# srtee/lammps-USER-CONP2

Measured on AMD Instinct MI355X. Metric: charge-solve updates/sec + ns/day, 4096-atom electrode / 32k electrolyte, higher is better.
Workload: dtype f64; 1 GPU; synthetic graphene/IL 4096 electrode + 32768 electrolyte, ffield; Ne=4096, Nl=32768, K=99773, kflat=645, mode=ffield, solver=inv, kspace=ewald, blist_pairs=302717, structure_factor_form=z-window (32 columns, grid 480)

## Files before the change

### include/conp_hip.h

```cpp
#ifndef CONP_HIP_H
#define CONP_HIP_H

#include <stddef.h>
#include <stdint.h>

#ifdef __cplusplus
extern "C" {
#endif

#define CONP_ABI_VERSION 1

typedef enum {
  CONP_OK = 0,
  CONP_ERR_ARG = -1,
  CONP_ERR_STATE = -2,
  CONP_ERR_NO_DEVICE = -3,
  CONP_ERR_NUMERIC = -4,
  CONP_ERR_IO = -5
} conp_status;

enum { CONP_FF_NORMAL = 0, CONP_FF_FFIELD = 1, CONP_FF_NOSLAB = 2 };
enum { CONP_SOLVER_CG = 0, CONP_SOLVER_INV = 1 };

typedef struct conp_fix conp_fix;
// ... 128 lines not shown
int conp_compute_potential_atom(conp_fix *fix, const conp_atoms *atoms, const conp_neighlist *pairlist, const int *sel,
                                const int *etasel , const conp_potential_args *args, double *potential);

typedef struct {
  int elenum, elenum_all, elytenum, maxtag_all, runstage;
  int kcount, kcount_flat, kcount_expand, kxmax, kymax, kzmax, kmax, kmax3d;
  int kcount_dims[7];
  int cg_iterations;
  int n_zclasses;
  double unitk[3], volume, gsqmx, ug_tot, totsetq, scalar_output, totinve, slabcorr;
  int64_t n_blist_pairs, n_alist_pairs, n_elyte_charged;
  int inverse_path;
  int inverse_retries;
  int pppm_elyte_spreads;
  int zn_cols, zn_grid, zn_rows;
} conp_info;
int conp_fix_info(const conp_fix *fix, conp_info *out);
int conp_fix_get_ktables(const conp_fix *fix, int *kxvecs, int *kyvecs, int *kzvecs, double *ug, int *kxy_list, int *kz_list);
int conp_fix_get_maps(const conp_fix *fix, int *ele2tag, int *ele2eleall, int *eleall2tag, int *eleall2ele,
                      int *elecheck_eleall, int *elebuf2eleall, int *tag2eleall);
int conp_fix_get_matrix(conp_fix *fix, double *aaa_all );
int conp_fix_set_matrix(conp_fix *fix, const double *aaa_all, int runstage);
int conp_fix_get_vectors(conp_fix *fix, double *bbb_all, double *eleallq, double *elesetq);
int conp_fix_get_sfac(conp_fix *fix, double *sfacrl, double *sfacim);
int conp_fix_get_ele_trig(conp_fix *fix, double *csk, double *snk);
int conp_inv_project(conp_fix *fix, int n, double *aaa, int nullneutral, int zneutr, const double *eleallz, double zhalf,
                     double *totinve_out);

int conp_fix_write_matrix_file(conp_fix *fix, const char *path, int which);
int conp_fix_read_matrix_file(conp_fix *fix, const conp_atoms *atoms, const char *path);
// ... 69 lines not shown
void conp_host_free(void *p);

int conp_debug_check_guards(void);

enum {
  CONP_PATH_PARTIAL_TILES = 1 << 0,
  CONP_PATH_A_GENERAL = 1 << 1,
  CONP_PATH_INV_PIVOTED = 1 << 2,
  CONP_PATH_CG_TWO_LAUNCH = 1 << 3,
  CONP_PATH_GEMV_ROWS = 1 << 4,
  CONP_PATH_PHASE_LAUNCH = 1 << 5,
  CONP_PATH_PPPM_SPREAD_LAUNCH = 1 << 6,
  CONP_PATH_ROWS_HOST = 1 << 7,
  CONP_PATH_TIME_SPLIT = 1 << 8,
  CONP_PATH_SK_CLASSIC = 1 << 12,
  CONP_PATH_ZN_WIDE = 1 << 13
};
void conp_debug_set_paths(unsigned mask);
void conp_debug_set_sk_workgroups(int n);
void conp_debug_set_ew_block(int n);


int conp_fix_write_timing(conp_fix *fix);
const char *conp_fix_log_drain(conp_fix *fix);
const char *conp_fix_mesg_drain(conp_fix *fix);

#ifdef __cplusplus
}
#endif
#endif
```

### lammps-user-conp2_amd/conp_amd/capi.py

```python
from __future__ import annotations

import ctypes as C
import os
from typing import Optional, Sequence

import numpy as np

from . import systems as _systems

HERE = os.path.dirname(os.path.abspath(__file__))
_LIB = None


class ConpError(RuntimeError):
    def __init__(self, code, msg):
        super().__init__(f"[conp status {code}] {msg}")
        self.code = code
        self.msg = msg


def library_path():
    return os.environ.get("CONP_LIB") or os.path.join(HERE, "libconp_hip.so")


# ... 49 lines not shown


class conp_pair_build_args(C.Structure):
    _fields_ = [("nlocal", C.c_int), ("nall", C.c_int), ("cutneigh", C.c_double), ("d_tag", C.c_void_p), ("d_nspecial", C.c_void_p),
                ("d_special", C.c_void_p), ("maxspecial", C.c_int), ("prd_half", C.c_double * 3)]


class conp_info(C.Structure):
    _fields_ = [("elenum", C.c_int), ("elenum_all", C.c_int), ("elytenum", C.c_int), ("maxtag_all", C.c_int),
                ("runstage", C.c_int), ("kcount", C.c_int), ("kcount_flat", C.c_int), ("kcount_expand", C.c_int),
                ("kxmax", C.c_int), ("kymax", C.c_int), ("kzmax", C.c_int), ("kmax", C.c_int), ("kmax3d", C.c_int),
                ("kcount_dims", C.c_int * 7), ("cg_iterations", C.c_int), ("n_zclasses", C.c_int), ("unitk", C.c_double * 3),
                ("volume", C.c_double), ("gsqmx", C.c_double), ("ug_tot", C.c_double), ("totsetq", C.c_double),
                ("scalar_output", C.c_double), ("totinve", C.c_double), ("slabcorr", C.c_double),
                ("n_blist_pairs", C.c_int64), ("n_alist_pairs", C.c_int64), ("n_elyte_charged", C.c_int64),
                ("inverse_path", C.c_int), ("inverse_retries", C.c_int), ("pppm_elyte_spreads", C.c_int), ("zn_cols", C.c_int), ("zn_grid", C.c_int), ("zn_rows", C.c_int)]


SYMBOLS = [
    "conp_parse_fix_args", "conp_fix_create", "conp_fix_destroy", "conp_last_error", "conp_abi_version",
    "conp_fix_init_list", "conp_fix_setup_post_neighbor", "conp_fix_setup_pre_force", "conp_fix_post_neighbor",
    "conp_fix_pre_force", "conp_fix_compute_scalar", "conp_fix_post_force", "conp_fix_post_force_step", "conp_fix_modify_param", "conp_fix_linalg_setup", "conp_fix_a_cal", "conp_fix_b_cal",
    "conp_fix_equation_solve", "conp_fix_update_charge", "conp_km_conp_setup", "conp_km_a_cal", "conp_km_b_cal",
    "conp_fix_info", "conp_fix_get_ktables", "conp_fix_get_maps", "conp_fix_get_matrix", "conp_fix_set_matrix",
    "conp_fix_get_vectors", "conp_fix_get_sfac", "conp_fix_get_ele_trig", "conp_inv_project", "conp_invert",
    "conp_host_ktables", "conp_host_index", "conp_host_pair_rows", "conp_fix_write_matrix_file", "conp_fix_read_matrix_file",
    "conp_fix_set_stream",
    "conp_fix_bind_device_buffers", "conp_fix_row_range", "conp_fix_b_cal_device", "conp_fix_solve_device",
    "conp_fix_scatter_device", "conp_fix_pre_force_device", "conp_fix_profile", "conp_fix_profile_read", "conp_debug_check_guards",
    "conp_debug_set_paths", "conp_debug_set_sk_workgroups", "conp_debug_set_ew_block",
    "conp_fix_pin_host_arrays", "conp_fix_unpin_host_arrays", "conp_host_alloc", "conp_host_free",
# ... 4 lines not shown
    "conp_ewald_compute", "conp_ewald_compute_group_potential", "conp_ewald_compute_particle_potential",
    "conp_ewald_compute_forces", "conp_pppm_compute_forces",
    "conp_ewald_compute_forces_device", "conp_pppm_compute_forces_device",
    "conp_ewald_compute_forces_vatom", "conp_pppm_compute_forces_vatom",
    "conp_ewald_compute_forces_vatom_device", "conp_pppm_compute_forces_vatom_device",
    "conp_compute_potential_atom",
    "conp_pair_set_params", "conp_pair_set_list", "conp_pair_compute", "conp_pair_compute_device",
    "conp_pair_build_list_device", "conp_pair_list_moved_device", "conp_pair_get_list",
]


PATH_PARTIAL_TILES, PATH_A_GENERAL, PATH_INV_PIVOTED, PATH_CG_TWO_LAUNCH, PATH_GEMV_ROWS = 1, 2, 4, 8, 16
PATH_PHASE_LAUNCH, PATH_PPPM_SPREAD_LAUNCH, PATH_ROWS_HOST, PATH_TIME_SPLIT = 32, 64, 128, 256
PATH_SK_CLASSIC = 4096
PATH_ZN_WIDE = 8192


class test_paths:

    def __init__(self, mask=0, sk_workgroups=0):
        self.mask, self.nwg = mask, sk_workgroups

    def __enter__(self):
        lib = load_library()
        if not hasattr(lib, "conp_debug_set_paths"):
            raise RuntimeError("this library build has no test hooks (a comparison build of an earlier round?)")
        lib.conp_debug_set_paths(self.mask)
        lib.conp_debug_set_sk_workgroups(self.nwg)
        return self

# ... 690 lines not shown
```

### lammps-user-conp2_amd/csrc/conp_fix.cpp

```cpp
#include <hip/hip_runtime.h>
#include <dlfcn.h>
#include <rccl/rccl.h>

#include <algorithm>
#include <cmath>
#include <cstdarg>
#include <chrono>
#include <cstdio>
#include <cstdlib>
#include <cstring>
#include <map>
#include <memory>
#include <mutex>
#include <stdexcept>
#include <string>
#include <vector>

#include "../../include/conp_hip.h"
#include "conp_host.hpp"
#include "conp_kernels.h"

namespace {

thread_local std::string g_last_error;
// ... 687 lines not shown
  bool zn_listed = false;
  bool zn_off = false;
  bool zn_tables_current = false;
  int zn_n = 0, zn_ncf = 2;
  double zn_gscale = 0.0, zn_beta = 0.0;
  std::vector<ZnItem> zn_items_h;
  DevBuf<ZnItem> d_zn_items;
  DevBuf<int> d_zn_g0c, d_zn_frag_ptr;
  DevBuf<int2> d_zn_frag_ents;
  DevBuf<double> d_zn_P, d_zn_phihat, d_zn_Bt, d_zn_pieces, d_zn_grid, d_zn_Dt;
  DevBuf<int> d_zn_cov_ptr;
  DevBuf<int2> d_zn_cov_ent;
  int zn_nrg = 0;
  DevBuf<double2> d_zn_cs;
  int zn_nfrag = 0;
  std::vector<int> zn_ch_lo, zn_ch_hi;
  int zn_c_start = 0;
  int *zn_flag_host = nullptr, *zn_flag_dev = nullptr;
  bool zn_eligible() const { return !decomposed && !args.pppm && nl >= zn_min_atoms && !path_on(CONP_PATH_SK_CLASSIC); }
  bool zn_use() const { return zn_listed && !zn_off && zn_eligible() && sk_projects() && nzc > 0; }
  bool zn_gen_use() const { return zn_listed && !zn_off && zn_eligible() && !sk_projects() && nzc == 0 && env.nranks <= 1 && zn_nrg > 0; }
  double zn_lz() const { return kt.slabflag ? env.zprd * env.slab_volfactor : env.zprd; }
  void zn_order_list(const conp_atoms *at) {
    zn_listed = false; zn_off = false;
    if (getenv("CONP_TIME_REN")) std::fprintf(stderr, "  z-window: eligible %d (decomposed %d pppm %d nl %d) plan.nz %d\n", (int)zn_eligible(), (int)decomposed, args.pppm, nl, plan.nz);
    if (!zn_eligible() || plan.nz <= 0) return;
    int n = std::max(64, (38 * plan.nz / 10 + 15) / 16 * 16);
    zn_n = n;
    zn_beta = 0.97 * 3.14159265358979323846 * ZN_W * (1.0 - (double)plan.nz / n);
    const double lz = zn_lz();
// ... 85 lines not shown
          if (pos[x] < per_xcd[x].size()) zn_items_h.push_back(by_slot[per_xcd[x][pos[x]++]]);
          else {
            int best = -1; size_t left = 0;
            for (int y = 0; y < 8; ++y) if (per_xcd[y].size() - pos[y] > left) { left = per_xcd[y].size() - pos[y]; best = y; }
            if (best >= 0) zn_items_h.push_back(by_slot[per_xcd[best][pos[best]++]]);
          }
    }
    zn_nfrag = 4 * plan.n_row_tiles;
    std::vector<std::vector<int2>> of_frag(zn_nfrag);
    for (const ZnItem &it : zn_items_h)
      for (int f = 0; f < 4; ++f) of_frag[4 * it.rt + f].push_back(make_int2(it.slot * sk_hc_stride() + 16 * f, 4));
    std::vector<int> fptr(zn_nfrag + 1, 0);
    std::vector<int2> fent;
    for (int g = 0; g < zn_nfrag; ++g) { fent.insert(fent.end(), of_frag[g].begin(), of_frag[g].end()); fptr[g + 1] = (int)fent.size(); }
    if (fent.empty()) fent.push_back(make_int2(0, 4));
    zn_nrg = nrg;
    if (nzc == 0) {
      const int ncol = 16 * zn_ncf;
      std::vector<int> cptr(n + 1, 0);
      std::vector<int2> cent;
      for (int g = 0; g < n; ++g) {
        for (int r = 0; r < nrg; ++r) {
          int col = (g - g0c[ranges[r].first]) % n;
          if (col < 0) col += n;
          if (col < ncol) cent.push_back(make_int2(r, col));
        }
        cptr[g + 1] = (int)cent.size();
      }
      if (cent.empty()) cent.push_back(make_int2(0, 0));
      ren_upload(d_zn_cov_ptr, cptr);
// ... 1014 lines not shown
        prof.begin("elyte_phase", stream);
        ZnWindow zw{};
        const bool zn_now = zn_use() || zn_gen_use();
        if (zn_now) zw = ZnWindow{d_zn_Bt.p, d_zn_g0c.p, zn_flag_dev, 16 * zn_ncf, zn_n, ZN_W, zn_beta, zn_gscale};
        launch_elyte_phase(stream, nl, nl_pad, eidx, ex, eq, kt.unitk[0], kt.unitk[1], kt.unitk[2], plan.kxmax,
                           plan.kymax, plan.nz, plan.kzt, 1 + plan.n_col_tiles * 32, d_Xt.p, d_Yt.p, d_Zt.p, d_qc.p, d_slab_part.p,
                           &n_slab_part, ride && !ride_hc ? &pairs : nullptr, d_breal.p, 16 * table_c0, 16 * table_c1, zn_now ? &zw : nullptr);
        zs_current = !zn_now; last_ex = ex; last_eq = eq; last_eidx = eidx;
        prof.end(stream);
        pairs_keep = pairs;
      }
      fin = make_brow(ne, ne_pad, rr0, rr1, d_b_rowptr.p, d_b_ele.p, d_b_oth.p, dx, dq, d_type.p, real_params(), 1, d_bk.p, slab,
                      d_ele_z.p, d_slab_part.p, n_slab_part, 4.0 * 3.14159265358979323846 / kt.volume, d_b, d_scalars.p + 2);
      fin.breal = d_breal.p;
      use_fin = ride && nzc > 0 && zc_final_fits((int)own_rt_h.size(), nzc);
      const bool proj = sk_projects();
      if (zn_use() && !fuse_phase) {
        zn_ensure_tables();
        prof.begin("zn_gemm", stream);
        launch_zn_gemm(stream, dplan, zn_ncf, d_zn_items.p, (int)zn_items_h.size(), d_Xt.p, d_Yt.p, d_zn_Bt.p, d_zn_P.p, zn_n, nzc,
                       d_zn_pieces.p, sk_hc_stride());
        prof.end(stream);
        g_current = false;
        prof.begin("reduce_project", stream);
        launch_project_zclass_pieces(stream, dplan, ne_pad, (int)own_rt_h.size(), d_own_rt.p, nzc, d_zn_pieces.p, d_hslot_ptr.p, d_hslot_idx.p,
                                     true, d_zn_frag_ptr.p, d_zn_frag_ents.p, zn_nfrag, d_Rp.p, d_Xe.p, d_Ye.p, d_own_pv.p, d_zclass.p, d_Hc.p,
                                     d_bk.p, use_fin ? &fin : nullptr, ride_hc ? &pairs_keep : nullptr, d_breal.p,
                                     zn_nrg > 32 );
        prof.end(stream);
      } else if (zn_gen_use() && !fuse_phase) {
        zn_ensure_tables();
        prof.begin("zn_gemm", stream);
        launch_zn_gemm(stream, dplan, zn_ncf, d_zn_items.p, (int)zn_items_h.size(), d_Xt.p, d_Yt.p, d_zn_Bt.p, nullptr, zn_n, 0,
                       d_zn_pieces.p, 0);
        prof.end(stream);
        prof.begin("sk_reduce", stream);
        launch_zn_windows_to_g(stream, dplan, plan.kzt, zn_n, (int)own_rt_h.size(), d_own_rt.p, zn_nrg, 16 * zn_ncf, d_zn_cov_ptr.p, d_zn_cov_ent.p,
                               d_zn_pieces.p, d_zn_grid.p, d_zn_Dt.p, d_G.p, d_Gw.p);
        prof.end(stream);
        g_current = true;
        prof.begin("b_project", stream);
        launch_b_project(stream, dplan, ne_pad, d_ct_ptr.p, d_tiles.p, d_Gw.p, d_Rp.p, d_Tz.p, d_bk.p);
        prof.end(stream);
// ... 917 lines not shown
  o->maxtag_all = f->idx.maxtag_all; o->runstage = f->runstage;
  o->kcount = f->kt.kcount; o->kcount_flat = f->kt.kcount_flat; o->kcount_expand = f->kt.kcount_expand;
  o->kxmax = f->kt.kxmax; o->kymax = f->kt.kymax; o->kzmax = f->kt.kzmax; o->kmax = f->kt.kmax; o->kmax3d = f->kt.kmax3d;
  for (int i = 0; i < 7; ++i) o->kcount_dims[i] = f->kt.kcount_dims[i];
  o->cg_iterations = f->cg_iterations;
  o->n_zclasses = f->nzc;
  for (int i = 0; i < 3; ++i) o->unitk[i] = f->kt.unitk[i];
  o->volume = f->kt.volume; o->gsqmx = f->kt.gsqmx; o->ug_tot = f->kt.ug_tot; o->totsetq = f->totsetq;
  o->scalar_output = f->scalar_output; o->totinve = f->totinve; o->slabcorr = f->slabcorr;
  int64_t nbp = f->n_b_pairs;
  if (f->np_pending) { HIP_TRY(hipStreamSynchronize(f->stream)); nbp = *f->h_np; }
  o->n_blist_pairs = nbp;
  o->inverse_path = f->inverse_path; o->inverse_retries = f->inverse_retries; o->pppm_elyte_spreads = f->pp_elyte_spreads;
  const bool zn_on = f->zn_use() || f->zn_gen_use();
  o->zn_cols = zn_on ? 16 * f->zn_ncf : 0; o->zn_grid = zn_on ? f->zn_n : 0; o->zn_rows = zn_on ? 128 * (int)f->own_rt_h.size() : 0; o->n_alist_pairs = f->arows.npairs(); o->n_elyte_charged = f->nl;
  CONP_GUARD_END
}

int conp_fix_get_ktables(const conp_fix *f, int *kx, int *ky, int *kz, double *ug, int *kxy_list, int *kz_list) {
  CONP_GUARD_BEGIN
  if (!f->kspace_ready) throw ConpError(CONP_ERR_STATE, "k tables not built");
  const size_t K = f->kt.kcount, E = f->kt.kcount_expand;
  if (kx) std::memcpy(kx, f->kt.kxvecs.data(), K * sizeof(int));
  if (ky) std::memcpy(ky, f->kt.kyvecs.data(), K * sizeof(int));
  if (kz) std::memcpy(kz, f->kt.kzvecs.data(), K * sizeof(int));
  if (ug) std::memcpy(ug, f->kt.ug.data(), K * sizeof(double));
  if (kxy_list) std::memcpy(kxy_list, f->kt.kxy_list.data(), E * sizeof(int));
  if (kz_list) std::memcpy(kz_list, f->kt.kz_list.data(), E * sizeof(int));
  CONP_GUARD_END
}
// ... 1234 lines not shown
```

### lammps-user-conp2_amd/csrc/conp_kernels.h

```cpp
#pragma once
#include <hip/hip_runtime.h>
#include <atomic>
#include <cstddef>
#include <cstdint>
#include "../../include/conp_hip.h"

namespace conp {

bool path_on(unsigned bit);
int debug_sk_workgroups();
int debug_ew_block();
const char *env_knob(const char *name);

struct DynLdsCache { std::atomic<size_t> granted[64]; };
template <typename K>
void ensure_dyn_lds(K kernel, size_t bytes, DynLdsCache &cache) {
  int dev = 0;
  (void)hipGetDevice(&dev);
  std::atomic<size_t> &g = cache.granted[dev & 63];
  if (bytes <= g.load(std::memory_order_relaxed)) return;
  if (hipFuncSetAttribute(reinterpret_cast<const void *>(kernel), hipFuncAttributeMaxDynamicSharedMemorySize, (int)bytes) == hipSuccess)
    g.store(bytes, std::memory_order_relaxed);
}

// ... 175 lines not shown
                        const BRowArgs *rows ,
                        double *breal_out, int j0 , int j1,
                        const ZnWindow *zw = nullptr );
bool zc_final_fits(int n_own, int nzc);
void launch_sk_gemm(hipStream_t s, const DevPlan &pl, const SkWItem *witems , int maxseg, int nwg, int nl_pad,
                    const double2 *Xt, const double2 *Yt, const double2 *Zs, const double *qc, double *part, const SkProj *proj = nullptr,
                    const SkFuse *fuse = nullptr ,
                    int fuse_rows = 0 );
int sk_hc_stride();
int sk_hc_max_classes();
void launch_project_zclass_pieces(hipStream_t s, const DevPlan &pl, int ne_pad, int n_own, const int *own_rt, int nzc, const double *Hp,
                                  const int *slot_ptr, const int *slot_idx, bool presum , const int *frag_ptr , const int2 *frag_ents , int nfrag, const double *Rp, const double2 *Xe,
                                  const double2 *Ye, const int *own_pv, const int *zclass, double *Hc, double *bk_part, const BRowArgs *fin,
                                  const BRowArgs *pairs = nullptr ,
                                  double *breal_out = nullptr,
                                  bool wide = false );
void launch_sk_reduce(hipStream_t s, const DevPlan &pl, const SkTile *tiles, int ntiles, int max_nsplit, double *part, double *G,
                      double *Gwf);
void launch_sfac_gather(hipStream_t s, int kcount, int C_pad, int PT, const int *sf_row_a, const int *sf_col_c,
                        const int *k_sign, const double *G, double *sfacrl, double *sfacim);
void launch_b_project(hipStream_t s, const DevPlan &pl, int ne_pad, const int *ct_ptr , const SkTile *tiles,
                      const double *Gwf, const double *Rp, const double *Tz, double *bk_part );
void launch_reduce_project_zclass(hipStream_t s, const DevPlan &pl, const SkTile *tiles, int ntiles, int max_nsplit, double *part,
                                  double *G, int ne_pad, int n_own, const int *own_rt, int nzc, const double *Tzc, const double *Rp,
                                  const double2 *Xe , const double2 *Ye ,
                                  const int *own_pv , const int *zclass, double *Hc, double *bk_part,
                                  const BRowArgs *fin );
void launch_b_project_zclass(hipStream_t s, const DevPlan &pl, int ne_pad, const int *rt_mine, int n_own, const int *own_rt, int nzc, const double *Gwf,
                             const double *Tzc , const double *Rp, const double2 *Xe, const double2 *Ye,
                             const int *own_pv, const int *zclass ,
                             double *Hc , double *bk_part , const BRowArgs *fin);
// ... 106 lines not shown
```

### lammps-user-conp2_amd/csrc/conp_kernels.hip

```cpp
#include "conp_kernels.h"
#include "conp_brow.hpp"

#include <atomic>
#include <cstdio>
#include <cstdlib>

namespace conp {

typedef double d4 __attribute__((ext_vector_type(4)));
#define MFMA_F64(a, b, c) __builtin_amdgcn_mfma_f64_16x16x4f64((a), (b), (c), 0, 0, 0)

const char *env_knob(const char *name) {
  const char *v = getenv(name);
  if (v) {
    static std::atomic<unsigned long long> said{0};
    unsigned h = 0;
    for (const char *c = name; *c; ++c) h = h * 31u + (unsigned char)*c;
    const unsigned long long bit = 1ull << (h & 63u);
    if (!(said.fetch_or(bit) & bit))
      fprintf(stderr, "libconp_hip: %s=%s is set -- a non-default code path is in use\n", name, v);
  }
  return v;
}
static std::atomic<unsigned> g_paths{0};
// ... 943 lines not shown
  for (; s + 8 <= s1; s += 8) {
    double v[8];
#pragma unroll
    for (int u = 0; u < 8; ++u) v[u] = h[(size_t)slot_idx[s + u] * stride];
    acc += ((v[0] + v[1]) + (v[2] + v[3])) + ((v[4] + v[5]) + (v[6] + v[7]));
  }
  double v[8];
#pragma unroll
  for (int u = 0; u < 8; ++u) v[u] = s + u < s1 ? h[(size_t)slot_idx[s + u] * stride] : 0.0;
  return acc + (((v[0] + v[1]) + (v[2] + v[3])) + ((v[4] + v[5]) + (v[6] + v[7])));
}

constexpr int HCS_MAXG = 16;
__global__ __launch_bounds__(256) void hc_sum_kernel(const int *__restrict__ frag_ptr, const int2 *__restrict__ ents, int R_pad, int nzc,
                                                     const double *__restrict__ Hp, double *__restrict__ Hc4, int nfrag, BRowArgs ra,
                                                     double *__restrict__ breal_out) {
  if ((int)blockIdx.y >= nfrag) {
    const int row = (((int)blockIdx.y - nfrag) * (int)gridDim.x + (int)blockIdx.x) * 4 + (int)(threadIdx.x >> 6);
    if (row < ra.ne) {
      const double v = b_row_pairs(ra, row, threadIdx.x & 63);
      if ((threadIdx.x & 63) == 0) breal_out[row] = v;
    }
    return;
  }
  const int g = blockIdx.y;
  const int s0 = frag_ptr[g], s1 = frag_ptr[g + 1];
  const int u = threadIdx.x & 7;
  const int e = blockIdx.x * 32 + (threadIdx.x >> 3);
  const bool live = e < 32 * nzc;
  const int cls = live ? e >> 5 : 0, half = (e >> 4) & 1, i = e & 15;
  double acc = 0.0;
  const int ng = (s1 - s0) / 8 + 1;
  for (int gb = 0; gb < ng; gb += HCS_MAXG) {
    double v[HCS_MAXG];
#pragma unroll
    for (int k = 0; k < HCS_MAXG; ++k) {
      const int sidx = s0 + 8 * (gb + k) + u;
      v[k] = 0.0;
      if (live && sidx < s1) {
        const int2 en = ents[sidx];
        v[k] = Hp[(size_t)en.x + (size_t)(cls * 32 * en.y + half * 16 * en.y + i)];
      }
    }
#pragma unroll
    for (int k = 0; k < HCS_MAXG; ++k) {
      if (gb + k >= ng) break;
      double t = v[k];
      t += __shfl_xor(t, 1, 64);
      t += __shfl_xor(t, 2, 64);
      t += __shfl_xor(t, 4, 64);
      acc += t;
    }
  }
  if (live && u == 0) Hc4[(size_t)cls * R_pad + (size_t)(g >> 2) * 128 + 64 * half + 16 * (g & 3) + i] = acc;
}

// ... 32 lines not shown
      }
    }
#pragma unroll
    for (int k = 0; k < 8; ++k) sum += rp[k] * hc[k];
  }
  red[w][a] = sum;
  __syncthreads();
  if (w == 0) {
    double tot = 0.0;
#pragma unroll
    for (int k = 0; k < 16; ++k) tot += red[k][a];
    bk[(size_t)blockIdx.y * ne_pad + i] = -tot;
  }
}

__global__ __launch_bounds__(1024) void b_zc_final_kernel(int n_own, const int *__restrict__ own_rt, int R_pad, int ne_pad, int nzc,
                                                          const double2 *__restrict__ Xe, const double2 *__restrict__ Ye,
                                                          const int *__restrict__ own_pv, const double *__restrict__ Hc4,
                                                          const int *__restrict__ zclass, BRowArgs ra, int nslot,
                                                          const int *__restrict__ slot_ptr, const int *__restrict__ slot_idx) {
#pragma clang fp contract(off)
  extern __shared__ __attribute__((aligned(16))) char zf_smem[];
  double *H = reinterpret_cast<double *>(zf_smem);
  __shared__ double red[64][17];
  const int a = threadIdx.x & 15, w = threadIdx.x >> 4;
  const int i = blockIdx.x * 16 + a;
  const int zc = zclass[i];
  const size_t hp = (size_t)R_pad * 64;
  const double sc = (ra.slab && threadIdx.x < 64) ? b_slab_scalar(ra, threadIdx.x) : 0.0;
  double fin_z = 0.0, fin_r = 0.0;
  if (w == 0 && i < ra.ne) { if (ra.slab) fin_z = ra.ele_z[i]; fin_r = ra.breal[i]; }
  double2 xe0[8], ye0[8];
  int sg0[8];
#pragma unroll
  for (int u = 0; u < 8; ++u) {
    const bool ok = u < n_own;
    const int pk = own_pv[(ok ? u : 0) * 64 + w];
    sg0[u] = (pk >> 24) & 1;
    xe0[u] = ok ? Xe[(size_t)(pk & 4095) * ne_pad + i] : make_double2(0.0, 0.0);
    ye0[u] = Ye[(size_t)((pk >> 12) & 4095) * ne_pad + i];
  }
  const int nrow = n_own * 128;
  if (slot_ptr) {
    for (int e = threadIdx.x; e < nrow * nzc; e += 1024) {
      const int cls = e / nrow, rowl = e - cls * nrow, k = rowl >> 7;
      H[rowl * nzc + cls] = hc_slot_sum(Hc4 + cls * 128 + (rowl & 127), slot_idx, slot_ptr[k], slot_ptr[k + 1], (size_t)SK_HC * SK_HC_ROWS);
    }
  } else
  for (int e = threadIdx.x; e < nrow * nzc; e += 1024) {
    const int cls = e / nrow, rowl = e - cls * nrow;
    const double *h = Hc4 + (size_t)cls * R_pad + (size_t)own_rt[rowl >> 7] * 128 + (rowl & 127);
    if (nslot == 1) { H[rowl * nzc + cls] = h[0]; continue; }
    const double h03 = (h[0] + h[hp]) + (h[2 * hp] + h[3 * hp]);
    H[rowl * nzc + cls] = nslot == 4 ? h03 : h03 + ((h[4 * hp] + h[5 * hp]) + (h[6 * hp] + h[7 * hp]));
  }
  __syncthreads();
  double sum = 0.0;
  auto phase = [](double2 X, double2 Y, int neg, double &pa, double &pb) {
    const double sy = neg ? -Y.y : Y.y;
    pa = X.x * Y.x - X.y * sy;
    pb = X.x * sy + X.y * Y.x;
  };
#pragma unroll
  for (int u = 0; u < 8; ++u) {
    const int kk = u < n_own ? u : 0;
    double pa, pb;
    phase(xe0[u], ye0[u], sg0[u], pa, pb);
    sum += pa * H[(kk * 128 + w) * nzc + zc];
    sum += pb * H[(kk * 128 + w + 64) * nzc + zc];
  }
  for (int k0 = 8; k0 < n_own; k0 += 4) {
    double2 xe[4], ye[4];
    int sg[4];
#pragma unroll
    for (int u = 0; u < 4; ++u) {
      const bool ok = k0 + u < n_own;
      const int pk = own_pv[(ok ? k0 + u : k0) * 64 + w];
      sg[u] = (pk >> 24) & 1;
      xe[u] = ok ? Xe[(size_t)(pk & 4095) * ne_pad + i] : make_double2(0.0, 0.0);
      ye[u] = Ye[(size_t)((pk >> 12) & 4095) * ne_pad + i];
    }
#pragma unroll
    for (int u = 0; u < 4; ++u) {
      const int kk = k0 + u < n_own ? k0 + u : k0;
      double pa, pb;
      phase(xe[u], ye[u], sg[u], pa, pb);
      sum += pa * H[(kk * 128 + w) * nzc + zc];
      sum += pb * H[(kk * 128 + w + 64) * nzc + zc];
    }
  }
  red[w][a] = sum;
  __syncthreads();
  if (w == 0 && i < ra.ne) {
    double tot = 0.0;
#pragma unroll
    for (int k = 0; k < 64; k += 4) tot += (red[k][a] + red[k + 1][a]) + (red[k + 2][a] + red[k + 3][a]);
    double v = -tot;
    if (ra.slab) v -= fin_z * sc;
    v += fin_r;
    ra.b_out[i] = v;
    if (ra.slab && i == 0 && ra.slab_out) *ra.slab_out = sc;
  }
}

constexpr int HCW_MAXK = 4;
template <int NO >
__global__ __launch_bounds__(256) void hc_sum_wide_kernel(const int *__restrict__ frag_ptr, const int2 *__restrict__ ents, int R_pad, int nzc,
                                                          const double *__restrict__ Hp, double *__restrict__ Hc4, int nfrag, BRowArgs ra,
                                                          double *__restrict__ breal_out) {
  if ((int)blockIdx.y >= nfrag) {
    const int row = (((int)blockIdx.y - nfrag) * (int)gridDim.x + (int)blockIdx.x) * 4 + (int)(threadIdx.x >> 6);
    if (row < ra.ne) {
      const double v = b_row_pairs(ra, row, threadIdx.x & 63);
      if ((threadIdx.x & 63) == 0) breal_out[row] = v;
    }
    return;
  }
  const int g = blockIdx.y;
  const int s0 = frag_ptr[g], s1 = frag_ptr[g + 1];
  const int u = threadIdx.x & 7, o = (threadIdx.x >> 3) & (NO - 1);
  const int e = blockIdx.x * (32 / NO) + threadIdx.x / (8 * NO);
  const bool live = e < 32 * nzc;
  const int cls = live ? e >> 5 : 0, half = (e >> 4) & 1, i = e & 15;
  const int lane = threadIdx.x & 63, lane0 = lane & ~(8 * NO - 1);
  double acc = 0.0;
  const int ng = (s1 - s0) / 8 + 1;
  for (int gb = 0; gb < ng; gb += NO * HCW_MAXK) {
    double t[HCW_MAXK];
#pragma unroll
    for (int k = 0; k < HCW_MAXK; ++k) {
      const int sidx = s0 + 8 * (gb + NO * k + o) + u;
      double v = 0.0;
      if (live && sidx < s1) {
        const int2 en = ents[sidx];
        v = Hp[(size_t)en.x + (size_t)(cls * 32 * en.y + half * 16 * en.y + i)];
      }
      t[k] = v;
    }
#pragma unroll
    for (int k = 0; k < HCW_MAXK; ++k) {
      double v = t[k];
      v += __shfl_xor(v, 1, 64);
      v += __shfl_xor(v, 2, 64);
      v += __shfl_xor(v, 4, 64);
      t[k] = v;
    }
#pragma unroll
    for (int k = 0; k < HCW_MAXK; ++k)
#pragma unroll
      for (int oo = 0; oo < NO; ++oo) {
        const double tv = __shfl(t[k], lane0 + 8 * oo, 64);
        if (gb + NO * k + oo < ng) acc += tv;
      }
  }
  if (live && (threadIdx.x & (8 * NO - 1)) == 0) Hc4[(size_t)cls * R_pad + (size_t)(g >> 2) * 128 + 64 * half + 16 * (g & 3) + i] = acc;
}


bool zc_final_fits(int n_own, int nzc) { return n_own > 0 && (size_t)n_own * 128 * nzc * sizeof(double) <= 64 * 1024; }

static void launch_b_zc_final(hipStream_t s, const DevPlan &pl, int n_own, const int *own_rt, int ne_pad, int nzc, const double2 *Xe,
                              const double2 *Ye, const int *own_pv, const double *Hc, const int *zclass, const BRowArgs &fin, int nslot,
                              const int *slot_ptr = nullptr, const int *slot_idx = nullptr) {
  const size_t lds = (size_t)n_own * 128 * nzc * sizeof(double);
  static DynLdsCache granted{};
  ensure_dyn_lds(b_zc_final_kernel, lds, granted);
  hipLaunchKernelGGL(b_zc_final_kernel, dim3(ne_pad / 16), dim3(1024), lds, s, n_own, own_rt, pl.R_pad, ne_pad, nzc, Xe, Ye, own_pv, Hc,
                     zclass, fin, nslot, slot_ptr, slot_idx);
}

static void launch_b_zc_dot(hipStream_t s, int n_own, const int *own_rt, int R_pad, int ne_pad, int nzc, const double *Rp,
                            const double *Hc, const int *zclass, double *bk_part, int nslot) {
  const size_t lds = (size_t)(n_own > 0 ? n_own : 1) * 32 * nzc * sizeof(double);
  static DynLdsCache granted{};
  ensure_dyn_lds(b_zc_dot_kernel, lds, granted);
  hipLaunchKernelGGL(b_zc_dot_kernel, dim3(ne_pad / 64, 4), dim3(1024), lds, s, n_own, own_rt, R_pad, ne_pad, nzc, Rp, Hc, zclass, bk_part, nslot);
}

template <int SKR_SL>
__global__ __launch_bounds__(SKR_T) void sk_reduce_hc_kernel(int C_pad, const SkTile *__restrict__ tiles, const double *__restrict__ part,
                                                           const double *__restrict__ wfull, double *__restrict__ G,
                                                           const double *__restrict__ Tzc ,
                                                           double *__restrict__ Hc4 , int R_pad, int nzc16,
// ... 70 lines not shown
  else launch_reduce_hc_sl<8>(s, pl, tiles, ntiles, max_nsplit, part, G, Tzc, Hc, nzc16);
  if (fin) launch_b_zc_final(s, pl, n_own, own_rt, ne_pad, nzc, Xe, Ye, own_pv, Hc, zclass, *fin, nslot);
  else launch_b_zc_dot(s, n_own, own_rt, pl.R_pad, ne_pad, nzc, Rp, Hc, zclass, bk_part, nslot);
}

void launch_b_project_zclass(hipStream_t s, const DevPlan &pl, int ne_pad, const int *rt_mine, int n_own, const int *own_rt, int nzc, const double *Gwf,
                             const double *Tzc, const double *Rp, const double2 *Xe, const double2 *Ye, const int *own_pv, const int *zclass,
                             double *Hc, double *bk_part, const BRowArgs *fin) {
  const int nzc16 = (nzc + 15) / 16;
  hipLaunchKernelGGL(b_hc_kernel, dim3(pl.R_pad / 16, 4), dim3(256), 0, s, pl.C_pad, pl.n_col_tiles, rt_mine, nzc16,
                     pl.nb_act, Gwf, Tzc, Hc, pl.R_pad);
  if (fin) launch_b_zc_final(s, pl, n_own, own_rt, ne_pad, nzc, Xe, Ye, own_pv, Hc, zclass, *fin, 4);
  else launch_b_zc_dot(s, n_own, own_rt, pl.R_pad, ne_pad, nzc, Rp, Hc, zclass, bk_part, 4);
}

void launch_project_zclass_pieces(hipStream_t s, const DevPlan &pl, int ne_pad, int n_own, const int *own_rt, int nzc, const double *Hp,
                                  const int *slot_ptr, const int *slot_idx, bool presum, const int *frag_ptr, const int2 *frag_ents, int nfrag,
                                  const double *Rp, const double2 *Xe,
                                  const double2 *Ye, const int *own_pv, const int *zclass, double *Hc, double *bk_part, const BRowArgs *fin,
                                  const BRowArgs *pairs, double *breal_out, bool wide) {
  if (n_own <= 0) return;
  if (fin && !presum) { launch_b_zc_final(s, pl, n_own, own_rt, ne_pad, nzc, Xe, Ye, own_pv, Hp, zclass, *fin, 0, slot_ptr, slot_idx); return; }
  if (nfrag > 0) {
    const BRowArgs ra = pairs ? *pairs : BRowArgs{};
    if (wide) {
      constexpr int NO = 4;
      const int extra = pairs ? ((ra.ne + 3) / 4 + NO * nzc - 1) / (NO * nzc) : 0;
      hipLaunchKernelGGL(hc_sum_wide_kernel<NO>, dim3(NO * nzc, nfrag + extra), dim3(256), 0, s, frag_ptr, frag_ents, pl.R_pad, nzc, Hp, Hc, nfrag, ra,
                         breal_out);
    } else {
      const int extra = pairs ? ((ra.ne + 3) / 4 + nzc - 1) / nzc : 0;
      hipLaunchKernelGGL(hc_sum_kernel, dim3(nzc, nfrag + extra), dim3(256), 0, s, frag_ptr, frag_ents, pl.R_pad, nzc, Hp, Hc, nfrag, ra, breal_out);
    }
  }
  if (fin) launch_b_zc_final(s, pl, n_own, own_rt, ne_pad, nzc, Xe, Ye, own_pv, Hc, zclass, *fin, 1);
  else launch_b_zc_dot(s, n_own, own_rt, pl.R_pad, ne_pad, nzc, Rp, Hc, zclass, bk_part, 1);
}

__global__ __launch_bounds__(256) void b_real_combine_kernel(BRowArgs a) {
  const int row = blockIdx.x * 4 + (threadIdx.x >> 6);
  if (row >= a.ne) return;
  const int lane = threadIdx.x & 63;
  const double sc = a.slab ? b_slab_scalar(a, lane) : 0.0;
  b_row(a, row, lane, sc);
}

void launch_b_real_combine(hipStream_t s, int ne, int ne_pad, int row0, int row1, const int *row_ptr, const int *ele_atom,
// ... 144 lines not shown
#pragma unroll
  for (int i = 0; i < 2; ++i) {
    const bool hi = lane & 8;
    const double keep = hi ? p[2 + i] : p[i], send = hi ? p[i] : p[2 + i];
    p[i] = keep + __shfl_xor(send, 8, 64);
  }
  {
    const bool hi = lane & 4;
    const double keep = hi ? p[1] : p[0], send = hi ? p[0] : p[1];
    p[0] = keep + __shfl_xor(send, 4, 64);
  }
  p[0] += __shfl_xor(p[0], 2, 64);
  return p[0] + __shfl_xor(p[0], 1, 64);
}

__global__ __launch_bounds__(256, 4) void sym_gemv_kernel(int ne, int ne_pad, const double *__restrict__ Spk, const double *__restrict__ b,
                                                          double *__restrict__ yp ) {
  __shared__ double bi_s[SG_T], bj_s[SG_T];
  __shared__ double tr[4][SG_T];
  int t = blockIdx.x, bi = 0;
  while ((bi + 1) * (bi + 2) / 2 <= t) ++bi;
  const int bj = t - bi * (bi + 1) / 2;
  const unsigned tid = threadIdx.x, lane = tid & 63, wave = tid >> 6;
  const double2 *tile = reinterpret_cast<const double2 *>(Spk + (size_t)t * SG_T * SG_T) + (size_t)(32 * wave) * 64 + lane;
  double2 v[16];
#pragma unroll
  for (int r = 0; r < 16; ++r) v[r] = tile[r * 64];
  {
    const int i = (tid < SG_T ? bi : bj) * SG_T + (int)(tid & (SG_T - 1));
    (tid < SG_T ? bi_s : bj_s)[tid & (SG_T - 1)] = i < ne ? b[i] : 0.0;
  }
  __syncthreads();
  const double bj0 = bj_s[2 * lane], bj1 = bj_s[2 * lane + 1];
  double at0 = 0.0, at1 = 0.0;
// ... 10 lines not shown
    }
    if (h == 0) {
      unsigned off2 = 16 * 64;
      asm volatile("" : "+v"(off2) : "v"(at0), "v"(at1));
#pragma unroll
      for (int r = 0; r < 16; ++r) v[r] = tile[off2 + r * 64];
    }
    const double rs = wave_sum16_transposed(p, lane);
    if ((lane & 3) == 0) ydir[16 * h] = rs;
  }
  if (bi != bj) {
    tr[wave][2 * lane] = at0; tr[wave][2 * lane + 1] = at1;
    __syncthreads();
    if (tid < SG_T) yp[(size_t)bi * ne_pad + bj * SG_T + tid] = (tr[0][tid] + tr[1][tid]) + (tr[2][tid] + tr[3][tid]);
  }
}

constexpr int SF_R = 32;
__global__ __launch_bounds__(4 * SF_R) void sym_finish_kernel(int n, int ne_pad, int nb, const double *__restrict__ yp, double *__restrict__ y,
                                                         const double *__restrict__ elesetq, const double *__restrict__ eleinitq,
                                                         double potdiff, const int *__restrict__ atoms_ptr,
                                                         const int *__restrict__ atoms_of, const int *__restrict__ atoms_row,
                                                         double *__restrict__ q_ele, double *__restrict__ q_atoms) {
  __shared__ double part[4][SF_R];
  __shared__ double vq[SF_R];
  const int rl = threadIdx.x & (SF_R - 1), g = threadIdx.x / SF_R;
  const int row0 = blockIdx.x * SF_R, row = row0 + rl;
  const int rend = row0 + SF_R < n ? row0 + SF_R : n;
  int k0 = 0, k1 = 0;
  if (q_atoms) { k0 = atoms_ptr[row0]; k1 = atoms_ptr[rend]; }
// ... 15 lines not shown
    const double r = (part[0][rl] + part[1][rl]) + (part[2][rl] + part[3][rl]);
    double v;
    {
#pragma clang fp contract(off)
      v = r + potdiff * sq;
      if (eleinitq) v += iq;
    }
    y[row] = r; q_ele[row] = v;
    vq[rl] = v;
  }
  __syncthreads();
  if (!q_atoms) return;
  for (int k = k0 + (int)threadIdx.x; k < k1; k += 4 * SF_R) q_atoms[atoms_of[k]] = vq[atoms_row[k] - row0];
}

size_t sym_packed_doubles(int ne_pad) { const size_t nb = ne_pad / SG_T; return nb * (nb + 1) / 2 * SG_T * SG_T; }
void launch_sym_pack(hipStream_t s, int ne, int ne_pad, const double *S, double *Spk, unsigned long long *stat) {
  const int nb = ne_pad / SG_T;
  (void)hipMemsetAsync(stat, 0, 2 * sizeof(unsigned long long), s);
  hipLaunchKernelGGL(sym_pack_kernel, dim3(nb * (nb + 1) / 2), dim3(256), 0, s, ne, S, Spk, stat);
}
void launch_sym_gemv_finish(hipStream_t s, int n, int ne_pad, const double *Spk, const double *b, double *yp, double *y,
                            const double *elesetq, const double *eleinitq, double potdiff, const int *atoms_ptr, const int *atoms_of,
                            const int *atoms_row, double *q_ele, double *q_atoms) {
  const int nb = ne_pad / SG_T;
  hipLaunchKernelGGL(sym_gemv_kernel, dim3(nb * (nb + 1) / 2), dim3(256), 0, s, n, ne_pad, Spk, b, yp);
  hipLaunchKernelGGL(sym_finish_kernel, dim3((n + SF_R - 1) / SF_R), dim3(4 * SF_R), 0, s, n, ne_pad, nb, (const double *)yp, y, elesetq, eleinitq,
                     potdiff, atoms_ptr, atoms_of, atoms_row, q_ele, q_atoms);
}

// ... 790 lines not shown
```

Baseline: 11690 updates/s.

## Stage phase rows in LDS for zc final and compute Hc fragment indices arithmetically

The zc-final kernel gets a templated staged variant that loads the small set of Xe/Ye phase rows for its 16-column block into LDS once, then reads per-pair phases from LDS instead of gathering from global memory, provided they fit within the LDS budget. The hc_sum kernels can also compute fragment entry offsets arithmetically when the host verifies that the fragment lists follow a regular pattern, which avoids the indirect ents table loads. It adds info fields, debug path switches and an optional sym_gemv timeline probe behind an ifdef. The cost is higher LDS use, which may lower occupancy for the final kernel.

```diff
diff --git a/include/conp_hip.h b/include/conp_hip.h
--- a/include/conp_hip.h
+++ b/include/conp_hip.h
@@ -166,6 +166,10 @@
   int inverse_retries;
   int pppm_elyte_spreads;
   int zn_cols, zn_grid, zn_rows;
+  int zn_ranges;
+  int hc_arithmetic;
+  int zc_final;
+  int zc_row_tiles;
 } conp_info;
 int conp_fix_info(const conp_fix *fix, conp_info *out);
 int conp_fix_get_ktables(const conp_fix *fix, int *kxvecs, int *kyvecs, int *kzvecs, double *ug, int *kxy_list, int *kz_list);
@@ -265,7 +269,9 @@
   CONP_PATH_ROWS_HOST = 1 << 7,
   CONP_PATH_TIME_SPLIT = 1 << 8,
   CONP_PATH_SK_CLASSIC = 1 << 12,
-  CONP_PATH_ZN_WIDE = 1 << 13
+  CONP_PATH_ZN_WIDE = 1 << 13,
+  CONP_PATH_ZC_PHASE_LOADS = 1 << 14,
+  CONP_PATH_HC_TABLES = 1 << 15
 };
 void conp_debug_set_paths(unsigned mask);
 void conp_debug_set_sk_workgroups(int n);
diff --git a/lammps-user-conp2_amd/conp_amd/capi.py b/lammps-user-conp2_amd/conp_amd/capi.py
--- a/lammps-user-conp2_amd/conp_amd/capi.py
+++ b/lammps-user-conp2_amd/conp_amd/capi.py
@@ -87,7 +87,8 @@
                 ("volume", C.c_double), ("gsqmx", C.c_double), ("ug_tot", C.c_double), ("totsetq", C.c_double),
                 ("scalar_output", C.c_double), ("totinve", C.c_double), ("slabcorr", C.c_double),
                 ("n_blist_pairs", C.c_int64), ("n_alist_pairs", C.c_int64), ("n_elyte_charged", C.c_int64),
-                ("inverse_path", C.c_int), ("inverse_retries", C.c_int), ("pppm_elyte_spreads", C.c_int), ("zn_cols", C.c_int), ("zn_grid", C.c_int), ("zn_rows", C.c_int)]
+                ("inverse_path", C.c_int), ("inverse_retries", C.c_int), ("pppm_elyte_spreads", C.c_int), ("zn_cols", C.c_int), ("zn_grid", C.c_int), ("zn_rows", C.c_int),
+                ("zn_ranges", C.c_int), ("hc_arithmetic", C.c_int), ("zc_final", C.c_int), ("zc_row_tiles", C.c_int)]
 
 
 SYMBOLS = [
@@ -122,6 +123,8 @@
 PATH_PHASE_LAUNCH, PATH_PPPM_SPREAD_LAUNCH, PATH_ROWS_HOST, PATH_TIME_SPLIT = 32, 64, 128, 256
 PATH_SK_CLASSIC = 4096
 PATH_ZN_WIDE = 8192
+PATH_ZC_PHASE_LOADS = 16384
+PATH_HC_TABLES = 32768
 
 
 class test_paths:
diff --git a/lammps-user-conp2_amd/csrc/conp_fix.cpp b/lammps-user-conp2_amd/csrc/conp_fix.cpp
--- a/lammps-user-conp2_amd/csrc/conp_fix.cpp
+++ b/lammps-user-conp2_amd/csrc/conp_fix.cpp
@@ -725,6 +725,8 @@
   int zn_nrg = 0;
   DevBuf<double2> d_zn_cs;
   int zn_nfrag = 0;
+  bool zn_frag_arith = false;
+  int zc_final_form = 0;
   std::vector<int> zn_ch_lo, zn_ch_hi;
   int zn_c_start = 0;
   int *zn_flag_host = nullptr, *zn_flag_dev = nullptr;
@@ -840,6 +842,7 @@
     std::vector<int2> fent;
     for (int g = 0; g < zn_nfrag; ++g) { fent.insert(fent.end(), of_frag[g].begin(), of_frag[g].end()); fptr[g + 1] = (int)fent.size(); }
     if (fent.empty()) fent.push_back(make_int2(0, 4));
+    zn_frag_arith = hc_frag_lists_arithmetic(fptr.data(), fent.data(), zn_nfrag, nrg, sk_hc_stride());
     zn_nrg = nrg;
     if (nzc == 0) {
       const int ncol = 16 * zn_ncf;
@@ -1884,6 +1887,7 @@
                       d_ele_z.p, d_slab_part.p, n_slab_part, 4.0 * 3.14159265358979323846 / kt.volume, d_b, d_scalars.p + 2);
       fin.breal = d_breal.p;
       use_fin = ride && nzc > 0 && zc_final_fits((int)own_rt_h.size(), nzc);
+      zc_final_form = !use_fin ? 0 : zc_final_phase_lds((int)own_rt_h.size(), nzc, plan.kxmax, plan.kymax) > 0 ? 2 : 1;
       const bool proj = sk_projects();
       if (zn_use() && !fuse_phase) {
         zn_ensure_tables();
@@ -1896,7 +1900,7 @@
         launch_project_zclass_pieces(stream, dplan, ne_pad, (int)own_rt_h.size(), d_own_rt.p, nzc, d_zn_pieces.p, d_hslot_ptr.p, d_hslot_idx.p,
                                      true, d_zn_frag_ptr.p, d_zn_frag_ents.p, zn_nfrag, d_Rp.p, d_Xe.p, d_Ye.p, d_own_pv.p, d_zclass.p, d_Hc.p,
                                      d_bk.p, use_fin ? &fin : nullptr, ride_hc ? &pairs_keep : nullptr, d_breal.p,
-                                     zn_nrg > 32 );
+                                     zn_nrg > 32 , zn_frag_arith ? zn_nrg : 0, sk_hc_stride());
         prof.end(stream);
       } else if (zn_gen_use() && !fuse_phase) {
         zn_ensure_tables();
@@ -2844,6 +2848,8 @@
   o->inverse_path = f->inverse_path; o->inverse_retries = f->inverse_retries; o->pppm_elyte_spreads = f->pp_elyte_spreads;
   const bool zn_on = f->zn_use() || f->zn_gen_use();
   o->zn_cols = zn_on ? 16 * f->zn_ncf : 0; o->zn_grid = zn_on ? f->zn_n : 0; o->zn_rows = zn_on ? 128 * (int)f->own_rt_h.size() : 0; o->n_alist_pairs = f->arows.npairs(); o->n_elyte_charged = f->nl;
+  o->zn_ranges = zn_on ? f->zn_nrg : 0; o->hc_arithmetic = f->zn_use() && f->zn_frag_arith ? 1 : 0;
+  o->zc_final = f->zc_final_form; o->zc_row_tiles = f->zc_final_form ? (int)f->own_rt_h.size() : 0;
   CONP_GUARD_END
 }
 
diff --git a/lammps-user-conp2_amd/csrc/conp_kernels.h b/lammps-user-conp2_amd/csrc/conp_kernels.h
--- a/lammps-user-conp2_amd/csrc/conp_kernels.h
+++ b/lammps-user-conp2_amd/csrc/conp_kernels.h
@@ -213,7 +213,11 @@
                                   const double2 *Ye, const int *own_pv, const int *zclass, double *Hc, double *bk_part, const BRowArgs *fin,
                                   const BRowArgs *pairs = nullptr ,
                                   double *breal_out = nullptr,
-                                  bool wide = false );
+                                  bool wide = false ,
+                                  int arith_nrg = 0 ,
+                                  int arith_stride = 0);
+bool hc_frag_lists_arithmetic(const int *frag_ptr, const int2 *ents, int nfrag, int nrg, int stride);
+size_t zc_final_phase_lds(int n_own, int nzc, int kxmax, int kymax);
 void launch_sk_reduce(hipStream_t s, const DevPlan &pl, const SkTile *tiles, int ntiles, int max_nsplit, double *part, double *G,
                       double *Gwf);
 void launch_sfac_gather(hipStream_t s, int kcount, int C_pad, int PT, const int *sf_row_a, const int *sf_col_c,
diff --git a/lammps-user-conp2_amd/csrc/conp_kernels.hip b/lammps-user-conp2_amd/csrc/conp_kernels.hip
--- a/lammps-user-conp2_amd/csrc/conp_kernels.hip
+++ b/lammps-user-conp2_amd/csrc/conp_kernels.hip
@@ -981,7 +981,7 @@
 constexpr int HCS_MAXG = 16;
 __global__ __launch_bounds__(256) void hc_sum_kernel(const int *__restrict__ frag_ptr, const int2 *__restrict__ ents, int R_pad, int nzc,
                                                      const double *__restrict__ Hp, double *__restrict__ Hc4, int nfrag, BRowArgs ra,
-                                                     double *__restrict__ breal_out) {
+                                                     double *__restrict__ breal_out, int nrg, int pstride) {
   if ((int)blockIdx.y >= nfrag) {
     const int row = (((int)blockIdx.y - nfrag) * (int)gridDim.x + (int)blockIdx.x) * 4 + (int)(threadIdx.x >> 6);
     if (row < ra.ne) {
@@ -991,7 +991,7 @@
     return;
   }
   const int g = blockIdx.y;
-  const int s0 = frag_ptr[g], s1 = frag_ptr[g + 1];
+  const int s0 = nrg > 0 ? (g >> 2) * nrg : frag_ptr[g], s1 = nrg > 0 ? s0 + nrg : frag_ptr[g + 1];
   const int u = threadIdx.x & 7;
   const int e = blockIdx.x * 32 + (threadIdx.x >> 3);
   const bool live = e < 32 * nzc;
@@ -1005,8 +1005,11 @@
       const int sidx = s0 + 8 * (gb + k) + u;
       v[k] = 0.0;
       if (live && sidx < s1) {
-        const int2 en = ents[sidx];
-        v[k] = Hp[(size_t)en.x + (size_t)(cls * 32 * en.y + half * 16 * en.y + i)];
+        if (nrg > 0) v[k] = Hp[(size_t)sidx * pstride + (size_t)(16 * (g & 3) + cls * 128 + half * 64 + i)];
+        else {
+          const int2 en = ents[sidx];
+          v[k] = Hp[(size_t)en.x + (size_t)(cls * 32 * en.y + half * 16 * en.y + i)];
+        }
       }
     }
 #pragma unroll
@@ -1069,14 +1072,17 @@
   }
 }
 
+template <bool STAGED>
 __global__ __launch_bounds__(1024) void b_zc_final_kernel(int n_own, const int *__restrict__ own_rt, int R_pad, int ne_pad, int nzc,
                                                           const double2 *__restrict__ Xe, const double2 *__restrict__ Ye,
                                                           const int *__restrict__ own_pv, const double *__restrict__ Hc4,
                                                           const int *__restrict__ zclass, BRowArgs ra, int nslot,
-                                                          const int *__restrict__ slot_ptr, const int *__restrict__ slot_idx) {
+                                                          const int *__restrict__ slot_ptr, const int *__restrict__ slot_idx,
+                                                          int nxr , int nyr ) {
 #pragma clang fp contract(off)
   extern __shared__ __attribute__((aligned(16))) char zf_smem[];
   double *H = reinterpret_cast<double *>(zf_smem);
+  double2 *PH = reinterpret_cast<double2 *>(zf_smem + (size_t)n_own * 128 * nzc * sizeof(double));
   __shared__ double red[64][17];
   const int a = threadIdx.x & 15, w = threadIdx.x >> 4;
   const int i = blockIdx.x * 16 + a;
@@ -1086,14 +1092,29 @@
   double fin_z = 0.0, fin_r = 0.0;
   if (w == 0 && i < ra.ne) { if (ra.slab) fin_z = ra.ele_z[i]; fin_r = ra.breal[i]; }
   double2 xe0[8], ye0[8];
-  int sg0[8];
-#pragma unroll
-  for (int u = 0; u < 8; ++u) {
-    const bool ok = u < n_own;
-    const int pk = own_pv[(ok ? u : 0) * 64 + w];
-    sg0[u] = (pk >> 24) & 1;
-    xe0[u] = ok ? Xe[(size_t)(pk & 4095) * ne_pad + i] : make_double2(0.0, 0.0);
-    ye0[u] = Ye[(size_t)((pk >> 12) & 4095) * ne_pad + i];
+  int pk0[8];
+  auto fetch = [&](int pk, bool ok, double2 &X, double2 &Y) {
+    if (STAGED) {
+      X = ok ? PH[(pk & 4095) * 16 + a] : make_double2(0.0, 0.0);
+      Y = PH[(nxr + ((pk >> 12) & 4095)) * 16 + a];
+    } else {
+      X = ok ? Xe[(size_t)(pk & 4095) * ne_pad + i] : make_double2(0.0, 0.0);
+      Y = Ye[(size_t)((pk >> 12) & 4095) * ne_pad + i];
+    }
+  };
+  auto row_elem = [&](int e) {
+    const int row = e >> 4;
+    const size_t col = (size_t)blockIdx.x * 16 + (e & 15);
+    return row < nxr ? Xe[(size_t)row * ne_pad + col] : Ye[(size_t)(row - nxr) * ne_pad + col];
+  };
+  const int nph = (nxr + nyr) * 16;
+#pragma unroll
+  for (int u = 0; u < 8; ++u) pk0[u] = own_pv[(u < n_own ? u : 0) * 64 + w];
+  double2 ph0 = make_double2(0.0, 0.0);
+  if (STAGED) { if ((int)threadIdx.x < nph) ph0 = row_elem(threadIdx.x); }
+  else {
+#pragma unroll
+    for (int u = 0; u < 8; ++u) fetch(pk0[u], u < n_own, xe0[u], ye0[u]);
   }
   const int nrow = n_own * 128;
   if (slot_ptr) {
@@ -1109,7 +1130,15 @@
     const double h03 = (h[0] + h[hp]) + (h[2 * hp] + h[3 * hp]);
     H[rowl * nzc + cls] = nslot == 4 ? h03 : h03 + ((h[4 * hp] + h[5 * hp]) + (h[6 * hp] + h[7 * hp]));
   }
-  __syncthreads();
+  if (STAGED) {
+    if ((int)threadIdx.x < nph) PH[threadIdx.x] = ph0;
+    for (int e = threadIdx.x + 1024; e < nph; e += 1024) PH[e] = row_elem(e);
+  }
+  __syncthreads();
+  if (STAGED) {
+#pragma unroll
+    for (int u = 0; u < 8; ++u) fetch(pk0[u], u < n_own, xe0[u], ye0[u]);
+  }
   double sum = 0.0;
   auto phase = [](double2 X, double2 Y, int neg, double &pa, double &pb) {
     const double sy = neg ? -Y.y : Y.y;
@@ -1120,7 +1149,7 @@
   for (int u = 0; u < 8; ++u) {
     const int kk = u < n_own ? u : 0;
     double pa, pb;
-    phase(xe0[u], ye0[u], sg0[u], pa, pb);
+    phase(xe0[u], ye0[u], (pk0[u] >> 24) & 1, pa, pb);
     sum += pa * H[(kk * 128 + w) * nzc + zc];
     sum += pb * H[(kk * 128 + w + 64) * nzc + zc];
   }
@@ -1132,8 +1161,7 @@
       const bool ok = k0 + u < n_own;
       const int pk = own_pv[(ok ? k0 + u : k0) * 64 + w];
       sg[u] = (pk >> 24) & 1;
-      xe[u] = ok ? Xe[(size_t)(pk & 4095) * ne_pad + i] : make_double2(0.0, 0.0);
-      ye[u] = Ye[(size_t)((pk >> 12) & 4095) * ne_pad + i];
+      fetch(pk, ok, xe[u], ye[u]);
     }
 #pragma unroll
     for (int u = 0; u < 4; ++u) {
@@ -1162,7 +1190,7 @@
 template <int NO >
 __global__ __launch_bounds__(256) void hc_sum_wide_kernel(const int *__restrict__ frag_ptr, const int2 *__restrict__ ents, int R_pad, int nzc,
                                                           const double *__restrict__ Hp, double *__restrict__ Hc4, int nfrag, BRowArgs ra,
-                                                          double *__restrict__ breal_out) {
+                                                          double *__restrict__ breal_out, int nrg, int pstride) {
   if ((int)blockIdx.y >= nfrag) {
     const int row = (((int)blockIdx.y - nfrag) * (int)gridDim.x + (int)blockIdx.x) * 4 + (int)(threadIdx.x >> 6);
     if (row < ra.ne) {
@@ -1172,7 +1200,7 @@
     return;
   }
   const int g = blockIdx.y;
-  const int s0 = frag_ptr[g], s1 = frag_ptr[g + 1];
+  const int s0 = nrg > 0 ? (g >> 2) * nrg : frag_ptr[g], s1 = nrg > 0 ? s0 + nrg : frag_ptr[g + 1];
   const int u = threadIdx.x & 7, o = (threadIdx.x >> 3) & (NO - 1);
   const int e = blockIdx.x * (32 / NO) + threadIdx.x / (8 * NO);
   const bool live = e < 32 * nzc;
@@ -1187,8 +1215,11 @@
       const int sidx = s0 + 8 * (gb + NO * k + o) + u;
       double v = 0.0;
       if (live && sidx < s1) {
-        const int2 en = ents[sidx];
-        v = Hp[(size_t)en.x + (size_t)(cls * 32 * en.y + half * 16 * en.y + i)];
+        if (nrg > 0) v = Hp[(size_t)sidx * pstride + (size_t)(16 * (g & 3) + cls * 128 + half * 64 + i)];
+        else {
+          const int2 en = ents[sidx];
+          v = Hp[(size_t)en.x + (size_t)(cls * 32 * en.y + half * 16 * en.y + i)];
+        }
       }
       t[k] = v;
     }
@@ -1213,15 +1244,28 @@
 
 
 bool zc_final_fits(int n_own, int nzc) { return n_own > 0 && (size_t)n_own * 128 * nzc * sizeof(double) <= 64 * 1024; }
+constexpr size_t ZF_DYN_LDS_MAX = 160 * 1024 - 64 * 17 * sizeof(double);
+size_t zc_final_phase_lds(int n_own, int nzc, int kxmax, int kymax) {
+  const size_t rows = (size_t)(kxmax + 2 + kymax + 1) * 16 * sizeof(double2);
+  if (path_on(CONP_PATH_ZC_PHASE_LOADS) || (size_t)n_own * 128 * nzc * sizeof(double) + rows > ZF_DYN_LDS_MAX) return 0;
+  return rows;
+}
 
 static void launch_b_zc_final(hipStream_t s, const DevPlan &pl, int n_own, const int *own_rt, int ne_pad, int nzc, const double2 *Xe,
                               const double2 *Ye, const int *own_pv, const double *Hc, const int *zclass, const BRowArgs &fin, int nslot,
                               const int *slot_ptr = nullptr, const int *slot_idx = nullptr) {
-  const size_t lds = (size_t)n_own * 128 * nzc * sizeof(double);
-  static DynLdsCache granted{};
-  ensure_dyn_lds(b_zc_final_kernel, lds, granted);
-  hipLaunchKernelGGL(b_zc_final_kernel, dim3(ne_pad / 16), dim3(1024), lds, s, n_own, own_rt, pl.R_pad, ne_pad, nzc, Xe, Ye, own_pv, Hc,
-                     zclass, fin, nslot, slot_ptr, slot_idx);
+  const size_t rows = zc_final_phase_lds(n_own, nzc, pl.kxmax, pl.kymax);
+  const size_t lds = (size_t)n_own * 128 * nzc * sizeof(double) + rows;
+  static DynLdsCache granted{}, granted_s{};
+  if (rows) {
+    ensure_dyn_lds(b_zc_final_kernel<true>, lds, granted_s);
+    hipLaunchKernelGGL(b_zc_final_kernel<true>, dim3(ne_pad / 16), dim3(1024), lds, s, n_own, own_rt, pl.R_pad, ne_pad, nzc, Xe, Ye, own_pv,
+                       Hc, zclass, fin, nslot, slot_ptr, slot_idx, pl.kxmax + 2, pl.kymax + 1);
+  } else {
+    ensure_dyn_lds(b_zc_final_kernel<false>, lds, granted);
+    hipLaunchKernelGGL(b_zc_final_kernel<false>, dim3(ne_pad / 16), dim3(1024), lds, s, n_own, own_rt, pl.R_pad, ne_pad, nzc, Xe, Ye, own_pv,
+                       Hc, zclass, fin, nslot, slot_ptr, slot_idx, pl.kxmax + 2, pl.kymax + 1);
+  }
 }
 
 static void launch_b_zc_dot(hipStream_t s, int n_own, const int *own_rt, int R_pad, int ne_pad, int nzc, const double *Rp,
@@ -1322,11 +1366,23 @@
   else launch_b_zc_dot(s, n_own, own_rt, pl.R_pad, ne_pad, nzc, Rp, Hc, zclass, bk_part, 4);
 }
 
+bool hc_frag_lists_arithmetic(const int *frag_ptr, const int2 *ents, int nfrag, int nrg, int stride) {
+  if (nrg <= 0 || nfrag <= 0 || path_on(CONP_PATH_HC_TABLES)) return false;
+  for (int g = 0; g < nfrag; ++g) {
+    if (frag_ptr[g] != g * nrg || frag_ptr[g + 1] != (g + 1) * nrg) return false;
+    for (int j = 0; j < nrg; ++j) {
+      const int2 en = ents[g * nrg + j];
+      if (en.y != 4 || (long long)en.x != ((long long)(g >> 2) * nrg + j) * stride + 16 * (g & 3)) return false;
+    }
+  }
+  return true;
+}
+
 void launch_project_zclass_pieces(hipStream_t s, const DevPlan &pl, int ne_pad, int n_own, const int *own_rt, int nzc, const double *Hp,
                                   const int *slot_ptr, const int *slot_idx, bool presum, const int *frag_ptr, const int2 *frag_ents, int nfrag,
                                   const double *Rp, const double2 *Xe,
                                   const double2 *Ye, const int *own_pv, const int *zclass, double *Hc, double *bk_part, const BRowArgs *fin,
-                                  const BRowArgs *pairs, double *breal_out, bool wide) {
+                                  const BRowArgs *pairs, double *breal_out, bool wide, int arith_nrg, int arith_stride) {
   if (n_own <= 0) return;
   if (fin && !presum) { launch_b_zc_final(s, pl, n_own, own_rt, ne_pad, nzc, Xe, Ye, own_pv, Hp, zclass, *fin, 0, slot_ptr, slot_idx); return; }
   if (nfrag > 0) {
@@ -1335,10 +1391,11 @@
       constexpr int NO = 4;
       const int extra = pairs ? ((ra.ne + 3) / 4 + NO * nzc - 1) / (NO * nzc) : 0;
       hipLaunchKernelGGL(hc_sum_wide_kernel<NO>, dim3(NO * nzc, nfrag + extra), dim3(256), 0, s, frag_ptr, frag_ents, pl.R_pad, nzc, Hp, Hc, nfrag, ra,
-                         breal_out);
+                         breal_out, arith_nrg, arith_stride);
     } else {
       const int extra = pairs ? ((ra.ne + 3) / 4 + nzc - 1) / nzc : 0;
-      hipLaunchKernelGGL(hc_sum_kernel, dim3(nzc, nfrag + extra), dim3(256), 0, s, frag_ptr, frag_ents, pl.R_pad, nzc, Hp, Hc, nfrag, ra, breal_out);
+      hipLaunchKernelGGL(hc_sum_kernel, dim3(nzc, nfrag + extra), dim3(256), 0, s, frag_ptr, frag_ents, pl.R_pad, nzc, Hp, Hc, nfrag, ra, breal_out, arith_nrg,
+                         arith_stride);
     }
   }
   if (fin) launch_b_zc_final(s, pl, n_own, own_rt, ne_pad, nzc, Xe, Ye, own_pv, Hc, zclass, *fin, 1);
@@ -1513,10 +1570,17 @@
   return p[0] + __shfl_xor(p[0], 1, 64);
 }
 
+#ifdef SYM_TIMELINE
+__device__ unsigned long long sym_tl[4096 * 3];
+#define SYM_STAMP(k) do { if (threadIdx.x == 0 && blockIdx.x < 4096) sym_tl[blockIdx.x * 3 + (k)] = wall_clock64(); } while (0)
+#else
+#define SYM_STAMP(k) do { } while (0)
+#endif
 __global__ __launch_bounds__(256, 4) void sym_gemv_kernel(int ne, int ne_pad, const double *__restrict__ Spk, const double *__restrict__ b,
                                                           double *__restrict__ yp ) {
   __shared__ double bi_s[SG_T], bj_s[SG_T];
   __shared__ double tr[4][SG_T];
+  SYM_STAMP(0);
   int t = blockIdx.x, bi = 0;
   while ((bi + 1) * (bi + 2) / 2 <= t) ++bi;
   const int bj = t - bi * (bi + 1) / 2;
@@ -1557,6 +1621,16 @@
     __syncthreads();
     if (tid < SG_T) yp[(size_t)bi * ne_pad + bj * SG_T + tid] = (tr[0][tid] + tr[1][tid]) + (tr[2][tid] + tr[3][tid]);
   }
+#ifdef SYM_TIMELINE
+  __syncthreads();
+  SYM_STAMP(1);
+  if (threadIdx.x == 0 && blockIdx.x < 4096) {
+    unsigned hw, xcc;
+    asm volatile("s_getreg_b32 %0, hwreg(HW_REG_HW_ID)" : "=s"(hw));
+    asm volatile("s_getreg_b32 %0, hwreg(HW_REG_XCC_ID)" : "=s"(xcc));
+    sym_tl[blockIdx.x * 3 + 2] = ((unsigned long long)xcc << 32) | hw;
+  }
+#endif
 }
 
 constexpr int SF_R = 32;
@@ -1602,6 +1676,11 @@
   for (int k = k0 + (int)threadIdx.x; k < k1; k += 4 * SF_R) q_atoms[atoms_of[k]] = vq[atoms_row[k] - row0];
 }
 
+#ifdef SYM_TIMELINE
+extern "C" int conp_debug_sym_timeline(unsigned long long *out, int nblocks) {
+  return (int)hipMemcpyFromSymbol(out, HIP_SYMBOL(sym_tl), sizeof(unsigned long long) * 3 * (size_t)nblocks);
+}
+#endif
 size_t sym_packed_doubles(int ne_pad) { const size_t nb = ne_pad / SG_T; return nb * (nb + 1) / 2 * SG_T * SG_T; }
 void launch_sym_pack(hipStream_t s, int ne, int ne_pad, const double *S, double *Spk, unsigned long long *stat) {
   const int nb = ne_pad / SG_T;
```

New measurement: 12100 updates/s, median of 6. 3.5% higher.
